# sanazkaviani/3d-latent-diffusion-model

Hardware: AMD Instinct MI355X
Metric: UNet denoising steps/sec (bf16, 1x4x24x24x24 latent; whole job = sum over GPUs) (higher is better)
Workload: dtype bf16

## Files before the change

3d-latent-diffusion-model_amd/csrc/ldm3d.hip:

```cpp
#include <hip/hip_runtime.h>
#include <dlfcn.h>
#include <math.h>
#include <stdarg.h>
#include <stdio.h>
#include <stdlib.h>
#include <string.h>

#include <algorithm>
#include <atomic>
#include <map>
#include <memory>
#include <string>
#include <vector>

#include "../../include/ldm3d.h"
#include "attention.h"
#include "conv_igemm.h"
#include "conv_halo.h"
#ifdef LDM_EXPERIMENTS
#include "conv_halo_pp.h"
#include "conv_halo_rw.h"
#endif
#include "conv_thin.h"
#include "gemm_light.h"
#include "gemm_light_x3.h"
#include "conv_block.h"
#include "conv_wgrad.h"
#include "conv_wgrad_w16.h"
#include "conv_wgrad_kw3.h"
#include "norm_elem.h"
#include "fin_gn.h"
#include "f32_path.h"
#include "f32_train.h"

#ifndef CONV_STAGES
#define CONV_STAGES 4
#endif

static thread_local char g_err[1024] = "";
static int fail(int code, const char* fmt, ...) {
    va_list ap; va_start(ap, fmt); vsnprintf(g_err, sizeof g_err, fmt, ap); va_end(ap);
    return code;
}
#define HIP_TRY(x) do { hipError_t e_ = (x); if (e_ != hipSuccess) \
    return fail(LDM_ERR_HIP, "%s failed: %s (%s:%d)", #x, hipGetErrorString(e_), __FILE__, __LINE__); } while (0)
#define LDM_TRY(x) do { int r_ = (x); if (r_ != 0) return r_; } while (0)


#ifdef LDM_EXPERIMENTS
static int g_block_slots = 0;
#endif
// ... 66 lines not shown
struct Ref { int base = BASE_NULL; size_t off = 0; };
static inline Ref ws_ref(size_t off) { Ref r; r.base = BASE_WS; r.off = off; return r; }
static inline Ref w_ref(size_t off) { Ref r; r.base = BASE_W; r.off = off; return r; }
static inline Ref io_ref(int i) { Ref r; r.base = BASE_IO0 + i; r.off = 0; return r; }
static inline Ref w32_ref(size_t off) { Ref r; r.base = BASE_W32; r.off = 2 * off; return r; }

struct Act {
    size_t off = 0; int C = 0; int N = 0, D = 0, H = 0, W = 0; bool valid = false;
    size_t stats_off = 0; bool has_stats = false;
    int stats_nrb = 0;
    int esz = 2;
    bool hl = false;
    size_t cs_off = 0; int cs_rows = 0;
    size_t bytes() const { return (size_t)N * D * H * W * C * esz; }
    long rows() const { return (long)N * D * H * W; }
};

enum OpKind { OP_PACK, OP_CONV, OP_FINALIZE, OP_GN_STATS, OP_GN_FINALIZE, OP_GN_PREP, OP_GN_APPLY, OP_ATTN, OP_SINUSOID,
              OP_GEMV, OP_VAE_HEADS, OP_GN_FUSED,
              OP_WT, OP_WT_BATCH, OP_WGRAD, OP_EXPORT, OP_EXPORT_BATCH, OP_COLSUM, OP_GNB, OP_ATTN_BWD, OP_ADD, OP_SUMPOOL, OP_LIN_DX, OP_LIN_DW, OP_VAE_HEADS_BWD,
              OP_GEMM_LIGHT,
              OP_COLSUM_BATCH,
              OP_IM2COL,
              OP_PACK32, OP_CONV32, OP_FIN32, OP_GN_STATS32, OP_GN_APPLY32, OP_ATTN32, OP_GEMV32,
              OP_TAP,
              OP_BUCKET, OP_BUCKET_JOIN,
              OP_UPS_SPLIT32,
              OP_CONV_THIN,
              OP_FIN_GN,
              OP_GEMM_LIGHT32,
              OP_CONV_BLOCK,
              OP_TEMB_ROW };

struct ConvCfg { int wgm, wgn, bk, splitk; int halo = 0, mtps = 0, qps = 0; int slab_lg = 0; };

struct Op {
    OpKind kind;
    Ref r[14];
    int i[24];
    float f[2];
    ConvCfg cc;
};

struct Pool {
    struct Blk { size_t off, size; };
    std::vector<Blk> free_list;
    std::map<size_t, size_t> live;
    size_t top = 0, high = 0;
    size_t alloc(size_t bytes) {
        bytes = rup_sz(bytes, 256);
        for (size_t k = 0; k < free_list.size(); ++k)
            if (free_list[k].size >= bytes) {
                size_t off = free_list[k].off;
                if (free_list[k].size == bytes) free_list.erase(free_list.begin() + k);
                else { free_list[k].off += bytes; free_list[k].size -= bytes; }
                live[off] = bytes;
                return off;
            }
        size_t off = top; top += bytes; high = std::max(high, top); live[off] = bytes;
        return off;
    }
    void release(size_t off) {
        auto it = live.find(off); if (it == live.end()) return;
        Blk b{off, it->second}; live.erase(it);
        free_list.push_back(b);
        std::sort(free_list.begin(), free_list.end(), [](const Blk& a, const Blk& c) { return a.off < c.off; });
        for (size_t k = 0; k + 1 < free_list.size();)
// ... 209 lines not shown
        a.valid = false; a.has_stats = false;
    }
    bool train = false, recording = false;

    struct ConvArgs {
        Act xa, xb;
        const ConvW* w = nullptr;
        int k = 3, stride = 1, pad = 1, ups = 0;
        int Do = 0, Ho = 0, Wo = 0;
        Act g1a, g1b; const ConvW* w1 = nullptr;
        Ref temb; int temb_stride = 0;
        Act residual;
        bool f32_out = false; Ref out_ref; int cout_real = 0;
        bool want_stats = true;
        Ref w_over; bool no_bias = false; int exact = 0;
        int temb_row = -1;
        int f32_tag = 0;
    };
    struct Tape {
        int kind = 0;
        ConvArgs c; Act out; bool leaf_input = false;
        const GnW* g = nullptr; Act xa, xb; size_t ab_off = 0, mr_off = 0; int groups = 0; bool silu = false;
        Act qkv, o; size_t lse_off = 0; int head_ch = 64;
    };
    std::vector<Tape> tape;

    static bool halo_enabled() { return ldm_knob("LDM_CONV_HALO", 1) != 0; }
    static int tall_mode() { return ldm_xknob("LDM_HALO_TALL", 2); }
    static bool light_enabled() { return ldm_knob("LDM_GEMM_LIGHT", 1) != 0; }
    static bool two_wg_enabled() { return ldm_knob("LDM_IGEMM_2WG", 1) != 0; }
    static bool phase_enabled() { return ldm_knob("LDM_CONV_PHASE", 1) != 0; }
    static bool halo_skip_enabled() { static const int v = ldm_knob("LDM_HALO_SKIP", 1); return v != 0; }
    static bool halo_skip_split_enabled() { static const int v = ldm_knob("LDM_HALO_SKIP_SPLIT", 1); return v != 0; }
    static ConvCfg choose_cfg(long M, int cout_pad, int steps0, int bk, int halo_n = 0, long halo_dhw = 0, bool halo_only = false, int steps1 = 0) {
        ConvCfg best{2, 2, bk, 1}; double best_t = 1e30;
        const int steps = steps0 + steps1;
        const int rb = bk * 2;
        static const int splits[] = {1, 2, 3, 4, 6, 8, 9, 12, 16, 18, 24, 27, 32, 48, 64};
        for (int wgn = 1; wgn <= 4 && !halo_only; wgn *= 2) {
            const int bn = 64 * wgn, bm = 64 * (4 / wgn);
            if (cout_pad % bn) continue;
            const long tiles = ((M + bm - 1) / bm) * (cout_pad / bn);
            const double c_mfma = (double)bm * bn * bk * 2.0 / 4096.0;
            const double c_load = (double)(bm + bn) * rb / 28.0;
            const double c_step = std::max(c_mfma, c_load) + 60.0;
            for (int sk : splits) {
                if (sk > 1 && steps / sk < 6) break;
                const long nwg = tiles * sk;
                const int sps = (steps + sk - 1) / sk;
                const double rounds = ceil((double)nwg / 256.0);
                double t = rounds * (sps * c_step + 2500.0);
                if (sk > 1) t += 6000.0 + (double)M * cout_pad * 4.0 * sk * 2.0 / 2500.0;
                if (t < best_t) { best_t = t; best = ConvCfg{4 / wgn, wgn, bk, sk}; }
            }
        }
        if (halo_n > 0 && bk == 64 && cout_pad % 128 == 0 && halo_enabled()) {
            const int mtps = (int)((halo_dhw + 125) / 126), Q = steps0 / 3;
            const long tiles = (long)halo_n * mtps * (cout_pad / 128);
            const double c_mfma = 128.0 * 128.0 * 64.0 * 2.0 / 4096.0;
            const double c_load = (128.0 / 3.0 + 128.0) * 128.0 / 28.0;
            const double c_step = std::max(c_mfma, c_load) + 30.0;
            for (int sk : splits) {
                if (sk > 1 && Q / sk < 3) break;
                const int qps = (Q + sk - 1) / sk, skr = (Q + qps - 1) / qps;
                const long nwg = tiles * skr;
                const double rounds = ceil((double)nwg / 256.0);
// ... 283 lines not shown
                Op op{}; op.kind = OP_CONV_BLOCK;
                op.r[0] = ws_ref(a.xa.off); op.r[2] = a.w_over.base != BASE_NULL ? a.w_over : w_ref(w.w_off); op.r[6] = a.no_bias ? Ref() : w_ref(w.b_off); op.r[8] = a.temb;
                op.r[9] = a.residual.valid ? ws_ref(a.residual.off) : Ref(); op.r[10] = ws_ref(out.off); op.r[12] = out.has_stats ? ws_ref(out.stats_off) : Ref();
                op.i[0] = N; op.i[1] = a.Do; op.i[2] = a.Ho; op.i[3] = a.Wo; op.i[4] = cin0; op.i[5] = TH; op.i[6] = a.temb_stride;
                plan->ops.push_back(op);
                if (recording) { Tape t; t.kind = 0; t.c = a; t.out = out; tape.push_back(t); }
                return out;
            }
        }
        if (conv_block128_enabled() && a.k == 3 && a.stride == 1 && a.pad == 1 && a.ups == 0 && !a.exact && !a.xb.valid && !a.w1 && !a.f32_out &&
            w.cout_pad == 128 && rup(w.cout, 32) == 128 && cin0 <= conv_block128_max_cin() && a.xa.D == a.Do && a.xa.H == a.Ho && a.xa.W == a.Wo) {
            const int td = (a.Do + BLK_TD - 1) / BLK_TD, th = (a.Ho + 7) / 8, tw = (a.Wo + BLK_TW - 1) / BLK_TW;
            static const long min_blocks = ldm_knob("LDM_CONV_BLOCK128_MIN", 192L);
            static const long max_blocks = ldm_xknob("LDM_CONV_BLOCK128_MAX", 0L);
            const long tiles128 = (long)N * td * th * tw;
            if (tiles128 >= min_blocks && tiles128 <= (max_blocks > 0 ? max_blocks : (long)device_cus())) {
                Act out = new_act(N, a.Do, a.Ho, a.Wo, 128);
                if (a.want_stats) { out.stats_off = pool.alloc((size_t)N * td * th * tw * 128 * 2 * 4); out.has_stats = true; out.stats_nrb = td * th * tw; }
                Op op{}; op.kind = OP_CONV_BLOCK;
                op.r[0] = ws_ref(a.xa.off); op.r[2] = a.w_over.base != BASE_NULL ? a.w_over : w_ref(w.w_off); op.r[6] = a.no_bias ? Ref() : w_ref(w.b_off); op.r[8] = a.temb;
                op.r[9] = a.residual.valid ? ws_ref(a.residual.off) : Ref(); op.r[10] = ws_ref(out.off); op.r[12] = out.has_stats ? ws_ref(out.stats_off) : Ref();
                op.i[0] = N; op.i[1] = a.Do; op.i[2] = a.Ho; op.i[3] = a.Wo; op.i[4] = cin0; op.i[5] = 8; op.i[6] = a.temb_stride; op.i[7] = 128;
                plan->ops.push_back(op);
                if (recording) { Tape t; t.kind = 0; t.c = a; t.out = out; tape.push_back(t); }
                return out;
            }
        }
        const int taps = phase ? 8 : a.k * a.k * a.k;
        const bool halo_ok = a.k == 3 && a.stride == 1 && a.pad == 1 && a.ups == 0 && !a.exact && !a.xb.valid && (!a.w1 || (halo_skip_enabled() && bk == 64)) &&
                             a.xa.D == a.Do && a.xa.H == a.Ho && a.xa.W == a.Wo;
        int nchunk0 = cin0 / bk, nchunk1 = cin1 / bk;
        int steps0 = taps * nchunk0, steps1 = nchunk1;
        ConvCfg cc = choose_cfg(M, w.cout_pad, steps0, bk, halo_ok ? N : 0, (long)a.Do * a.Ho * a.Wo, false, steps1);
        const int bm = 64 * cc.wgm, bn = 64 * cc.wgn;
        const int couts = a.f32_out ? 0 : rup(w.cout, 32);
        const int mtiles_pp = (int)(((long)a.xa.D * a.xa.H * a.xa.W + bm - 1) / bm);
        if (!cc.halo && cc.bk == 64 && cc.wgm <= 2 && cc.splitk == 1 && two_wg_enabled() && steps0 + steps1 <= 64 &&
            (phase ? (long)N * 8 * mtiles_pp : (M + bm - 1) / bm) * (w.cout_pad / bn) >= 512) {
            cc.bk = 32; nchunk0 = cin0 / 32; nchunk1 = cin1 / 32; steps0 = taps * nchunk0; steps1 = nchunk1;
        }
        Act out;
        if (!a.f32_out) {
            out = new_act(N, a.Do, a.Ho, a.Wo, couts);
            if (a.want_stats) {
                const long dhwo = (long)a.Do * a.Ho * a.Wo;
                if (cc.splitk > 1) {
                    out.stats_off = pool.alloc((size_t)((M + 31) / 32) * couts * 2 * 4); out.has_stats = true; out.stats_nrb = 0;
                } else if (cc.halo) {
                    out.stats_off = pool.alloc((size_t)N * cc.mtps * couts * 2 * 4); out.has_stats = true; out.stats_nrb = cc.mtps;
                } else if (phase) {
                    out.stats_off = pool.alloc((size_t)N * 8 * mtiles_pp * couts * 2 * 4); out.has_stats = true; out.stats_nrb = 8 * mtiles_pp;
                } else if (N == 1 || dhwo % bm == 0) {
                    out.stats_off = pool.alloc((size_t)((M + bm - 1) / bm) * couts * 2 * 4); out.has_stats = true;
                    out.stats_nrb = (int)(N == 1 ? (M + bm - 1) / bm : dhwo / bm);
                }
            }
        }
        Op op{}; op.kind = OP_CONV; op.cc = cc;
        op.r[0] = ws_ref(a.xa.off); op.r[1] = a.xb.valid ? ws_ref(a.xb.off) : Ref();
        op.r[2] = a.w_over.base != BASE_NULL ? a.w_over : w_ref(phase ? w.wp_off : w.w_off);
        op.r[3] = a.w1 ? ws_ref(a.g1a.off) : Ref(); op.r[4] = (a.w1 && a.g1b.valid) ? ws_ref(a.g1b.off) : Ref();
        op.r[5] = a.w1 ? w_ref(a.w1->w_off) : Ref();
        op.r[6] = a.no_bias ? Ref() : w_ref(w.b_off); op.r[7] = a.w1 ? w_ref(a.w1->b_off) : Ref();
        op.r[8] = a.temb; op.r[9] = a.residual.valid ? ws_ref(a.residual.off) : Ref();
        op.r[10] = a.f32_out ? a.out_ref : ws_ref(out.off);
        op.r[11] = Ref();
// ... 1155 lines not shown
            HIP_TRY(hipFuncSetAttribute(reinterpret_cast<const void*>(&conv3_halo_rw_kernel<0>), hipFuncAttributeMaxDynamicSharedMemorySize, HRW_LDS));
            HIP_TRY(hipFuncSetAttribute(reinterpret_cast<const void*>(&conv3_halo_rw_kernel<64>), hipFuncAttributeMaxDynamicSharedMemorySize, HRW_LDS));
            HIP_TRY(hipFuncSetAttribute(reinterpret_cast<const void*>(&conv3_halo_rw_kernel<4>), hipFuncAttributeMaxDynamicSharedMemorySize, HRW_LDS));
            rw_attr = true;
        }
        if ((p.dbg & 124) == 64) { hipLaunchKernelGGL((conv3_halo_rw_kernel<64>), dim3(tiles), dim3(512), HRW_LDS, s, p); return 0; }
        if ((p.dbg & 124) == 4) { hipLaunchKernelGGL((conv3_halo_rw_kernel<4>), dim3(tiles), dim3(512), HRW_LDS, s, p); return 0; }
        hipLaunchKernelGGL((conv3_halo_rw_kernel<0>), dim3(tiles), dim3(512), HRW_LDS, s, p);
        return 0;
    }
#endif
    if (p.dbg & (4 | 8 | 16 | 32 | 64 | 128 | 256)) {
#define ABL_CASE(A) if ((p.dbg & 508) == A) { \
            HIP_TRY(hipFuncSetAttribute(reinterpret_cast<const void*>(&conv3_halo_kernel<6, A>), hipFuncAttributeMaxDynamicSharedMemorySize, LDS)); \
            hipLaunchKernelGGL((conv3_halo_kernel<6, A>), dim3(p.mtiles * p.ntiles * p.splitk), dim3(512), LDS, s, p); return 0; }
        if ((p.dbg & 508) == 384) {
            constexpr int LDSX = LDS + 64;
            if (p.dbg & 2048) {
                HIP_TRY(hipFuncSetAttribute(reinterpret_cast<const void*>(&conv3_halo_kernel<6, 385>), hipFuncAttributeMaxDynamicSharedMemorySize, LDSX));
                hipLaunchKernelGGL((conv3_halo_kernel<6, 385>), dim3(p.mtiles * p.ntiles * p.splitk), dim3(512), LDSX, s, p); return 0;
            }
            HIP_TRY(hipFuncSetAttribute(reinterpret_cast<const void*>(&conv3_halo_kernel<6, 384>), hipFuncAttributeMaxDynamicSharedMemorySize, LDSX));
            hipLaunchKernelGGL((conv3_halo_kernel<6, 384>), dim3(p.mtiles * p.ntiles * p.splitk), dim3(512), LDSX, s, p); return 0;
        }
        ABL_CASE(4) ABL_CASE(8) ABL_CASE(16) ABL_CASE(12) ABL_CASE(20) ABL_CASE(24) ABL_CASE(32) ABL_CASE(40) ABL_CASE(84) ABL_CASE(68) ABL_CASE(64) ABL_CASE(128) ABL_CASE(256)
#undef ABL_CASE
    }
    if (loop) hipLaunchKernelGGL((conv3_halo_kernel<6, 0, false, true>), dim3(grid), dim3(512), LDS, s, p);
    else if (mi) hipLaunchKernelGGL((conv3_halo_kernel<6, 0, false, false, true>), dim3(grid), dim3(512), LDS, s, p);
    else hipLaunchKernelGGL((conv3_halo_kernel<6>), dim3(grid), dim3(512), LDS, s, p);
    return 0;
}

static int launch_conv_impl(const ConvParams& p, const ConvCfg& cc, hipStream_t s) {
    if (cc.halo) return launch_conv_halo(p, s, cc.halo == 2);
#define CASE(M_, N_, K_) if (cc.wgm == M_ && cc.wgn == N_ && cc.bk == K_) return launch_conv_t<M_, N_, K_>(p, s);
    CASE(2, 2, 64) CASE(4, 1, 64) CASE(1, 4, 64) CASE(2, 2, 32) CASE(4, 1, 32) CASE(1, 4, 32)
#undef CASE
    return fail(LDM_ERR_BAD_ARG, "no conv kernel for tile config %dx%d bk %d", cc.wgm, cc.wgn, cc.bk);
}

static inline int grid_for(long total, int per_block = 256, int cap = 4096) {
    long g = (total + per_block - 1) / per_block; if (g > cap) g = cap; if (g < 1) g = 1; return (int)g;
}

static void conv32_cfg(long M, int cout_pad, int steps, bool x3, int* bn_out, int* sk_out) {
    static const int f32_bn = ldm_knob("LDM_F32_BN", 0);
    static const int f32_wgs = ldm_knob("LDM_F32_WGS", 512);
    const int mtiles = (int)((M + 127) / 128);
    int bn = (cout_pad % 128) ? 64 : 128;
    if (f32_bn == 64 || (f32_bn == 1 && (long)mtiles * (cout_pad / 128) < 256)) bn = 64;
    const long tiles = (long)mtiles * ((cout_pad + bn - 1) / bn);
    int sk = 1;
    if (tiles < f32_wgs * 3 / 4) {
        sk = (int)std::min<long>(std::max<long>(1, f32_wgs / tiles), std::max(1, steps / (x3 ? 4 : 8)));
        const int sps = (steps + sk - 1) / sk; sk = (steps + sps - 1) / sps;
    }
    *bn_out = bn; *sk_out = sk;
}
static int fin32_stats_blocks(int N, int dhwo, int couts, int* rows) {
    const int cvec = couts / 4, rows_par = std::max(1, 256 / cvec);
    int nrb = std::min((dhwo + rows_par - 1) / rows_par, std::max(1, 256 / N));
    *rows = (dhwo + nrb - 1) / nrb;
    return (dhwo + *rows - 1) / *rows;
}
static void launch_conv32(const Conv32Params& p, bool x3, int bn, hipStream_t s) {
    const dim3 grid(p.mtiles * p.ntiles * p.splitk);
// ... 89 lines not shown
    static const int w16 = ldm_knob("LDM_WGRAD_W16", 1);
    if (w16 && p.pair == 0) {
        static bool attr16_tab[32] = {}; bool& attr16 = attr_flag(attr16_tab);
        if (!attr16) { HIP_TRY(hipFuncSetAttribute(reinterpret_cast<const void*>(&conv_wgrad_w16_kernel<0>), hipFuncAttributeMaxDynamicSharedMemorySize, LDS)); attr16 = true; }
        hipLaunchKernelGGL(conv_wgrad_w16_kernel<0>, dim3(p.co_tiles * p.ci_tiles * tg_ * p.ksplit), dim3(1024), LDS, s, p);
        return 0;
    }
    hipLaunchKernelGGL(conv_wgrad_kernel<0>, dim3(p.co_tiles * p.ci_tiles * tg_ * p.ksplit), dim3(512), LDS, s, p);
    return 0;
}

static bool wt_stores() { static const int v = ldm_xknob("LDM_WT_STORES", 1); return v != 0; }

struct PlanTrace { bool on = false; std::string path; PlanTrace() { const char* e = getenv("LDM_PLAN_TRACE"); if (e && *e) { on = true; path = e; } } };
static PlanTrace g_plan_trace;
struct LaneCtx { GradSyncState* sync = nullptr; };

static int run_plan(const Plan& plan, const Bases& bs, const int* rt, hipStream_t s, size_t begin = 0, size_t end = (size_t)-1,
                    LaneCtx lanes = LaneCtx()) {
    if (end > plan.ops.size()) end = plan.ops.size();
    const char* trace_path = g_plan_trace.on ? g_plan_trace.path.c_str() : nullptr;
    std::vector<hipEvent_t> tev;
    if (trace_path) { tev.resize(end - begin + 1); for (auto& e : tev) HIP_TRY(hipEventCreate(&e)); }
    struct TraceDone {
        const Plan& plan; size_t begin, end; std::vector<hipEvent_t>& ev; hipStream_t s; const char* path;
        ~TraceDone() {
            if (ev.empty()) return;
            (void)hipEventRecord(ev.back(), s); (void)hipEventSynchronize(ev.back());
            FILE* f = fopen(path, "a");
            for (size_t oi = begin; oi < end && f; ++oi) {
                const Op& o = plan.ops[oi]; float ms = 0.f; (void)hipEventElapsedTime(&ms, ev[oi - begin], ev[oi - begin + 1]);
                fprintf(f, "%zu,%zu,%d,%.3f", plan.ops.size(), oi, (int)o.kind, ms * 1e3f);
                if (o.kind == OP_CONV || o.kind == OP_FINALIZE)
                    fprintf(f, ",M=%d k=%d s=%d ups=%d cin=%d+%d(x%d) cin1=%d couts=%d cfg=%dx%dx%d splitk=%d halo=%d mtps=%d qps=%d", o.i[15], o.i[11], o.i[12],
                            o.i[14], o.i[0], o.i[1], o.i[19], o.i[2] + o.i[3], o.i[16], o.cc.wgm, o.cc.wgn, o.cc.bk, o.cc.splitk, o.cc.halo, o.cc.mtps, o.cc.qps);
                else fprintf(f, ",i=%d %d %d %d %d %d", o.i[0], o.i[1], o.i[2], o.i[3], o.i[4], o.i[5]);
                fprintf(f, "\n");
            }
            if (f) fclose(f);
            for (auto e : ev) (void)hipEventDestroy(e);
        }
    } trace_done{plan, begin, end, tev, s, trace_path};
    for (size_t oi = begin; oi < end; ++oi) {
        const Op& o = plan.ops[oi];
        const int* i = o.i;
        if (trace_path) HIP_TRY(hipEventRecord(tev[oi - begin], s));
        switch (o.kind) {
            case OP_PACK: {
                const long total = (long)i[0] * i[3] * i[2];
                int cx = rt[0], cc = rt[1];
                if (i[4]) { cx = i[1]; cc = 0; }
                if (cx + cc != i[1]) return fail(LDM_ERR_BAD_ARG, "x_channels + cond_channels = %d, model expects %d", cx + cc, i[1]);
                hipLaunchKernelGGL(pack2_ncdhw_kernel, dim3(grid_for(total)), dim3(256), 0, s, (const float*)rp(bs, o.r[0]), cx,
                                   (const float*)rp(bs, o.r[1]), cc, (bf16_t*)rp(bs, o.r[2]), i[0], i[2], i[3]);
                break; }
            case OP_IM2COL: {
                int cx = rt[0], cc = rt[1];
                if (i[6]) { cx = i[1]; cc = 0; }
                if (cx + cc != i[1]) return fail(LDM_ERR_BAD_ARG, "x_channels + cond_channels = %d, model expects %d", cx + cc, i[1]);
                const long total = (long)i[0] * i[3] * i[4] * i[5] * (i[2] / 8);
                hipLaunchKernelGGL(pack_im2col_kernel, dim3(grid_for(total, 256, 16384)), dim3(256), 0, s, (const float*)rp(bs, o.r[0]), cx,
                                   (const float*)rp(bs, o.r[1]), cc, (bf16_t*)rp(bs, o.r[2]), i[0], i[3], i[4], i[5], i[2]);
                break; }
            case OP_CONV_THIN: {
                ThinParams q{}; q.x = (const bf16_t*)rp(bs, o.r[0]); q.w = (const bf16_t*)rp(bs, o.r[2]); q.bias = (const float*)rp(bs, o.r[6]);
                q.out = (float*)rp(bs, o.r[10]); q.N = i[0]; q.D = i[1]; q.H = i[2]; q.W = i[3]; q.Cin = i[4]; q.CoutPad = i[5]; q.CoutReal = i[6];
                q.x3_c = i[7];
                if (!q.w) return fail(LDM_ERR_NOT_LOADED, "the weight arena is empty");
// ... 1129 lines not shown
    for (auto& e : g_prof.ev) HIP_TRY(hipEventCreate(&e));
    g_prof.wgm = wgm; g_prof.wgn = wgn; g_prof.bk = bk & 0xff; g_prof.halo = (bk >> 8) & 1; g_prof.on = true;
    return 0;
}
int ldm_profile_detail(double* flops, double* ms, int max) {
    if (!flops || !ms || max < 0) return fail(LDM_ERR_BAD_ARG, "null argument");
    const int n = (int)(g_prof.used / 2);
    for (int k = 0; k < n && k < max; ++k) {
        HIP_TRY(hipEventSynchronize(g_prof.ev[2 * k + 1]));
        float t = 0.f; HIP_TRY(hipEventElapsedTime(&t, g_prof.ev[2 * k], g_prof.ev[2 * k + 1]));
        flops[k] = g_prof.flops[k]; ms[k] = t;
    }
    return n;
}
int ldm_profile_stop(double out[5]) {
    if (!out) return fail(LDM_ERR_BAD_ARG, "null out");
    g_prof.on = false;
    double ms = 0.0, fl = 0.0;
    for (size_t k = 0; k + 1 < g_prof.used + 1 && k < g_prof.used; k += 2) {
        HIP_TRY(hipEventSynchronize(g_prof.ev[k + 1]));
        float t = 0.f; HIP_TRY(hipEventElapsedTime(&t, g_prof.ev[k], g_prof.ev[k + 1]));
        ms += t; fl += g_prof.flops[k / 2];
    }
    out[0] = (double)(g_prof.used / 2); out[1] = ms; out[2] = fl; out[3] = (double)g_prof.launches_all; out[4] = g_prof.flops_all;
    for (auto e : g_prof.ev) (void)hipEventDestroy(e);
    g_prof.ev.clear(); g_prof.used = 0; g_prof.flops.clear();
    return 0;
}
int ldm_model_plan_conv_cfgs(ldm_model* m, const char* kind, int B, int D, int H, int W, int* cfgs, int max_convs) {
    if (!m || !kind) return fail(LDM_ERR_BAD_ARG, "null argument");
    std::shared_ptr<Plan> p; LDM_TRY(get_plan(m, kind, B, D, H, W, &p));
    int n = 0;
    for (const Op& o : p->ops) if (o.kind == OP_CONV) {
        if (cfgs && n < max_convs) { cfgs[4 * n] = o.cc.wgm; cfgs[4 * n + 1] = o.cc.wgn; cfgs[4 * n + 2] = o.cc.bk | (o.cc.halo << 8); cfgs[4 * n + 3] = o.cc.splitk; }
        ++n;
    } else if (o.kind == OP_CONV_BLOCK) {
        if (cfgs && n < max_convs) { cfgs[4 * n] = 4; cfgs[4 * n + 1] = o.i[7] == 128 ? 2 : 1; cfgs[4 * n + 2] = 32 | ((o.i[7] == 128 ? 4 : 3) << 8); cfgs[4 * n + 3] = 1; }
        ++n;
    }
    return n;
}

int ldm_model_plan_launches(ldm_model* m, const char* kind, int B, int D, int H, int W) {
    if (!m || !kind) return fail(LDM_ERR_BAD_ARG, "null argument");
    std::shared_ptr<Plan> p; LDM_TRY(get_plan(m, kind, B, D, H, W, &p));
    int n = 0;
    for (const Op& o : p->ops) if (o.kind != OP_TAP) ++n;
    return n;
}

static char* g_zero_page = nullptr;
static int ensure_zero_page() {
    if (g_zero_page) return 0;
    HIP_TRY(hipMalloc((void**)&g_zero_page, 8192));
    HIP_TRY(hipMemset(g_zero_page, 0, 8192));
    HIP_TRY(hipDeviceSynchronize());
    return 0;
}

int ldm_op_conv3d_block128(const void* x, int cin, const void* w, const float* bias, const float* temb, int temb_stride, const void* residual,
                           void* out, float* stats, int N, int D, int H, int W, void* stream) {
    if (!x || !w || !out || N < 1 || D < 1 || H < 1 || W < 1 || cin < 32 || cin % 32) return fail(LDM_ERR_BAD_ARG, "bad argument");
    if ((long)N * D * H * W * cin * 2 >= (1L << 32)) return fail(LDM_ERR_BAD_ARG, "the input tensor exceeds 4 GiB (split the batch)");
    BlockParams q{}; q.x = (const bf16_t*)x; q.w = (const bf16_t*)w; q.bias = bias; q.temb = temb; q.temb_stride = temb_stride;
    q.residual = (const bf16_t*)residual; q.out = (bf16_t*)out; q.stats = stats; q.N = N; q.D = D; q.H = H; q.W = W; q.Cin = cin;
    HIP_TRY(launch_conv_block128(q, (hipStream_t)stream));
    return 0;
// ... 41 lines not shown
    int bk = 64;
    if (ca % 64 || cb % 64 || c1a % 64 || c1b % 64) bk = 32;
    const int Du = Din << ups, Hu = Hin << ups, Wu = Win << ups;
    const int pad_total = (stride == 2 && pad == 0 && ksize == 3) ? 1 : 2 * pad;
    const int Do = (Du + pad_total - ksize) / stride + 1, Ho = (Hu + pad_total - ksize) / stride + 1,
              Wo = (Wu + pad_total - ksize) / stride + 1;
    const long M = (long)N * Do * Ho * Wo;
    if (M >= (1L << 31) || M < 1) return fail(LDM_ERR_BAD_ARG, "bad output size");
    if (!stats && !wgn && !splitk && out_bf16 && !out_f32 && gemm_light_ok(ksize, stride, ups, cin0, cin1 == 0, !temb && !bias2) &&
        Builder::light_enabled() && M * (long)cin0 * 2 < (1L << 31)) {
        LightParams lp{}; lp.x = (const bf16_t*)xa; lp.w = (const bf16_t*)w; lp.bias = bias; lp.residual = (const bf16_t*)residual;
        lp.out = (bf16_t*)out_bf16; lp.stats = nullptr; lp.M = (int)M; lp.K = cin0; lp.CoutS = rup(cout, 32);
        lp.xb = (const bf16_t*)xb; lp.ca = ca;
        HIP_TRY(launch_gemm_light(lp, cout_pad, gemm_light_big(M, cout_pad), (hipStream_t)stream));
        return 0;
    }
    const int taps = ksize * ksize * ksize;
    ConvParams p{};
    p.x0a = (const bf16_t*)xa; p.x0b = (const bf16_t*)xb; p.c0a = ca; p.c0b = cb; p.w0 = (const bf16_t*)w;
    p.x1a = (const bf16_t*)x1a; p.x1b = (const bf16_t*)x1b; p.c1a = c1a; p.c1b = c1b; p.w1 = (const bf16_t*)w1;
    p.zero_page = (const bf16_t*)g_zero_page;
    p.N = N; p.Din = Din; p.Hin = Hin; p.Win = Win; p.Dout = Do; p.Hout = Ho; p.Wout = Wo;
    p.ksize = ksize; p.stride = stride; p.pad = pad; p.ups = ups; p.exact = exact; p.M = (int)M;
    p.CoutS = rup(cout, 32); p.CoutPad = cout_pad; p.CoutReal = cout;
    p.nchunk0 = cin0 / bk; p.nchunk1 = cin1 / bk; p.steps0 = taps * p.nchunk0; p.steps1 = p.nchunk1;
    const bool halo_ok = ksize == 3 && stride == 1 && pad == 1 && ups == 0 && !exact && cb == 0 && bk == 64 &&
                         (cin1 == 0 || (Builder::halo_skip_enabled() && (splitk <= 1 || Builder::halo_skip_split_enabled()))) && Builder::halo_enabled();
    ConvCfg cc = Builder::choose_cfg(M, cout_pad, p.steps0, bk, halo_ok ? N : 0, (long)Do * Ho * Wo, false, p.steps1);
    if (wgn) {
        if ((wgn != 1 && wgn != 2 && wgn != 4) || cout_pad % (64 * wgn)) return fail(LDM_ERR_BAD_ARG, "bad wgn");
        cc.wgn = wgn; cc.wgm = 4 / wgn; cc.halo = (wgn == 2 && halo_ok && cout_pad % 128 == 0) ? 1 : (wgn == 1 && halo_ok && Builder::tall_mode() != 0) ? 2 : 0;
    }
    if (splitk) cc.splitk = splitk;
    if (cc.splitk < 1 || cc.splitk > p.steps0 + p.steps1) return fail(LDM_ERR_BAD_ARG, "bad splitk");
    if (cc.halo) {
        const int Q = 9 * p.nchunk0;
        if (cc.splitk > Q) cc.splitk = Q;
        cc.qps = (Q + cc.splitk - 1) / cc.splitk; cc.splitk = (Q + cc.qps - 1) / cc.qps;
        cc.mtps = (int)(((long)Do * Ho * Wo + (cc.halo == 2 ? 253 : 125)) / (cc.halo == 2 ? 254 : 126));
    }
    p.splitk = cc.splitk; p.steps_per_split = cc.halo ? 3 * cc.qps : (p.steps0 + p.steps1 + cc.splitk - 1) / cc.splitk;
    p.halo_mtps = cc.mtps; p.q_per_split = cc.qps;
    p.mtiles = cc.halo ? N * cc.mtps : (int)((M + 64 * cc.wgm - 1) / (64 * cc.wgm)); p.ntiles = cout_pad / (64 * cc.wgn);
    p.bias = bias; p.bias2 = bias2; p.temb = temb; p.temb_stride = temb_stride; p.residual = (const bf16_t*)residual;
    p.out = out_f32 ? nullptr : (bf16_t*)out_bf16; p.out_f32 = out_f32;
    if (cc.splitk > 1) {
        const size_t need = (size_t)cc.splitk * M * cout_pad * 4;
        if (!scratch || scratch_bytes < need) return fail(LDM_ERR_WORKSPACE, "split-K scratch too small: need %zu bytes", need);
        p.partial = (float*)scratch;
    }
    if (stats) {
        const long dhwo = (long)Do * Ho * Wo; const int bm = 64 * cc.wgm;
        if (out_f32 || !stats_nrb) return fail(LDM_ERR_BAD_ARG, "statistics need the bf16 output form");
        if (cc.splitk > 1) { if (N > 1 && dhwo % 32) return fail(LDM_ERR_UNSUPPORTED, "statistics: DHW %% 32 != 0 with a batch"); *stats_nrb = (int)(N == 1 ? (M + 31) / 32 : dhwo / 32); }
        else if (cc.halo) *stats_nrb = cc.mtps;
        else { if (N > 1 && dhwo % bm) return fail(LDM_ERR_UNSUPPORTED, "statistics: tiles straddle samples"); *stats_nrb = (int)(N == 1 ? (M + bm - 1) / bm : dhwo / bm); }
        p.stats = stats;
    }
    p.dbg = (int)ldm_xknob("LDM_CONV_DBG", 0);
    if (p.dbg & 512) {
        if (cc.splitk > 1 || !scratch || scratch_bytes < (size_t)p.mtiles * p.ntiles * (64 + 4096)) return fail(LDM_ERR_BAD_ARG, "stamps need scratch and splitk 1");
        p.stamps = (unsigned long long*)scratch;
    }
    if (fg && cc.splitk > 1) p.slab_lg = fg->lg;
    LDM_TRY(launch_conv(p, cc, (hipStream_t)stream));
    if (cc.splitk > 1) {
        FinalizeParams f{}; f.partial = p.partial; f.splitk = p.splitk; f.M = p.M; f.CoutPad = p.CoutPad; f.CoutS = p.CoutS;
        f.CoutReal = p.CoutReal; f.DHWo = Do * Ho * Wo; f.bias = bias; f.bias2 = bias2; f.temb = temb; f.temb_stride = temb_stride;
// ... 768 lines not shown
```

Baseline: 492.9.

## Add whole-cube split-K conv kernel for tiny 3D volumes (edge at most 6)

Adds a specialized 3x3x3 conv kernel for tiny spatial volumes (at most 6^3). Each workgroup loads the whole zero-padded cube for one 64-channel input slice plus all 27 taps of weights into LDS in a single pass. It then runs all taps from LDS, adds any skip-input GEMM, and writes split-K partials. It targets the bottleneck-resolution convs, where the generic igemm/halo tiling leaves most of each tile empty and pays repeated load stalls. In exchange it needs a split-K finalize pass over an fp32 partial buffer, and runs one workgroup per CU with a large LDS footprint.

```diff
diff --git a/3d-latent-diffusion-model_amd/csrc/conv_cube.h b/3d-latent-diffusion-model_amd/csrc/conv_cube.h
--- /dev/null
+++ b/3d-latent-diffusion-model_amd/csrc/conv_cube.h
@@ -0,0 +1,171 @@
+#pragma once
+#include "conv_igemm.h"
+
+constexpr int CUBE_EDGE = 6;
+constexpr int CUBE_RP = 7, CUBE_PP = 49;
+constexpr int CUBE_ROWS = 448;
+constexpr int CUBE_TILES = 16;
+constexpr int CUBE_WOFF = 8 * CUBE_ROWS * 16;
+constexpr int CUBE_SOFF = CUBE_WOFF + 27 * 2048;
+constexpr int CUBE_SWOFF = CUBE_SOFF + 8 * 256 * 16;
+constexpr int CUBE_LDS = CUBE_SWOFF + 2048;
+static_assert(CUBE_LDS <= 160 * 1024, "LDS budget");
+static_assert(CUBE_ROWS % 64 == 0 && CUBE_ROWS % 16 == 0, "whole LDS-DMA copies; chunk stride a multiple of 16 rows");
+
+__device__ __forceinline__ void cube_vm_wait(int n) {
+    switch (n) {
+    case 0: asm volatile("s_waitcnt vmcnt(0)" ::: "memory"); break;
+    case 8: asm volatile("s_waitcnt vmcnt(8)" ::: "memory"); break;
+    case 9: asm volatile("s_waitcnt vmcnt(9)" ::: "memory"); break;
+    default: asm volatile("s_waitcnt vmcnt(0)" ::: "memory"); break;
+    }
+}
+__device__ __forceinline__ void cube_barrier() {
+    asm volatile("s_waitcnt lgkmcnt(0)" ::: "memory");
+    __builtin_amdgcn_s_barrier();
+    asm volatile("" ::: "memory");
+}
+
+__global__ __launch_bounds__(256, 1) __attribute__((amdgpu_waves_per_eu(1, 1))) void conv3_cube_kernel(const ConvParams p) {
+#if defined(__HIP_DEVICE_COMPILE__)
+    extern __shared__ __attribute__((aligned(16))) char smem[];
+    typedef __attribute__((address_space(3))) void* lds_ptr_t;
+    constexpr unsigned OOB = 0x80000000u;
+    KSTAMP_BEGIN(12);
+    const int tid = threadIdx.x, lane = tid & 63;
+    const int wave = __builtin_amdgcn_readfirstlane(tid >> 6);
+    const int split = blockIdx.x, n0 = blockIdx.y * 16, smp = blockIdx.z;
+    const int D = p.Dout, H = p.Hout, W = p.Wout, DHW = D * H * W, dom = D * H * CUBE_RP;
+    const unsigned cin2 = (unsigned)p.c0a * 2u, ci2 = (unsigned)split * 128u;
+
+    {
+        __amdgpu_buffer_rsrc_t rs_w = __builtin_amdgcn_make_buffer_rsrc((void*)p.w0, 0, (int)(27u * (unsigned)p.CoutPad * cin2), 0x00020000);
+        const int co = lane & 15, cq = lane >> 4;
+        for (int u = wave; u < 54; u += 4) {
+            const int tap = u >> 1, ch = (u & 1) * 4 + cq;
+            const unsigned vo = (unsigned)(tap * p.CoutPad + n0 + co) * cin2 + ci2 + (unsigned)ch * 16u;
+            __builtin_amdgcn_raw_ptr_buffer_load_lds(rs_w, (lds_ptr_t)(smem + CUBE_WOFF + u * 1024), 16, vo, 0, 0, 0);
+        }
+    }
+    {
+        const bf16_t* xs = p.x0a + (size_t)smp * DHW * p.c0a;
+        __amdgpu_buffer_rsrc_t rs_x = __builtin_amdgcn_make_buffer_rsrc((void*)xs, 0, (int)((unsigned)DHW * cin2), 0x00020000);
+        for (int v = wave; v < 8 * (CUBE_ROWS / 64); v += 4) {
+            const int ch = v / (CUBE_ROWS / 64), r = (v - ch * (CUBE_ROWS / 64)) * 64 + lane;
+            const int dp = r / CUBE_PP, rem = r - dp * CUBE_PP, hp = rem / CUBE_RP, wp = rem - hp * CUBE_RP;
+            const bool real = dp >= 1 && dp <= D && hp >= 1 && hp <= H && wp >= 1 && wp <= W;
+            const unsigned vo = real ? (unsigned)(((dp - 1) * H + hp - 1) * W + wp - 1) * cin2 + ci2 + (unsigned)ch * 16u : OOB;
+            __builtin_amdgcn_raw_ptr_buffer_load_lds(rs_x, (lds_ptr_t)(smem + ch * (CUBE_ROWS * 16) + (v - ch * (CUBE_ROWS / 64)) * 1024), 16, vo, 0, 0, 0);
+        }
+    }
+    int j0 = 0, j1 = 0;
+    if (p.steps1 > 0) {
+        const int per = (p.steps1 + p.splitk - 1) / p.splitk;
+        j0 = split * per; j1 = j0 + per; if (j1 > p.steps1) j1 = p.steps1; if (j0 > j1) j0 = j1;
+    }
+    unsigned s_vox = OOB;
+    {
+        const int q = wave * 64 + lane;
+        if (q < dom) {
+            const int d = q / (H * CUBE_RP), rem = q - d * H * CUBE_RP, h = rem / CUBE_RP, w = rem - h * CUBE_RP;
+            if (w < W) s_vox = (unsigned)((d * H + h) * W + w);
+        }
+    }
+    const int nca = p.c1a / 64;
+    const unsigned w1row2 = (unsigned)(p.c1a + p.c1b) * 2u;
+    auto issue_skip = [&](const int j) {
+        const bool a = j < nca;
+        const bf16_t* src = (a ? p.x1a : p.x1b) + (size_t)smp * DHW * (a ? p.c1a : p.c1b);
+        const unsigned row2 = (unsigned)(a ? p.c1a : p.c1b) * 2u, jc = (unsigned)(a ? j : j - nca) * 128u;
+        __amdgpu_buffer_rsrc_t rs_s = __builtin_amdgcn_make_buffer_rsrc((void*)src, 0, (int)((unsigned)DHW * row2), 0x00020000);
+#pragma unroll
+        for (int i = 0; i < 8; ++i) {
+            const unsigned vo = s_vox != OOB ? s_vox * row2 + jc + (unsigned)i * 16u : OOB;
+            __builtin_amdgcn_raw_ptr_buffer_load_lds(rs_s, (lds_ptr_t)(smem + CUBE_SOFF + i * 4096 + wave * 1024), 16, vo, 0, 0, 0);
+        }
+        if (wave < 2) {
+            __amdgpu_buffer_rsrc_t rs_1w = __builtin_amdgcn_make_buffer_rsrc((void*)p.w1, 0, (int)((unsigned)p.CoutPad * w1row2), 0x00020000);
+            const unsigned vo = (unsigned)(n0 + (lane & 15)) * w1row2 + (unsigned)j * 128u + (unsigned)(wave * 4 + (lane >> 4)) * 16u;
+            __builtin_amdgcn_raw_ptr_buffer_load_lds(rs_1w, (lds_ptr_t)(smem + CUBE_SWOFF + wave * 1024), 16, vo, 0, 0, 0);
+        }
+    };
+    const bool has_skip = j1 > j0;
+    if (has_skip) issue_skip(j0);
+    const int skip_copies = 8 + (wave < 2 ? 1 : 0);
+
+    const int mh = wave & 1, kh = wave >> 1;
+    const int fr = lane & 15, ch = kh * 4 + (lane >> 4);
+    int abase[8];
+#pragma unroll
+    for (int t = 0; t < 8; ++t) {
+        const int q = (mh * 8 + t) * 16 + fr;
+        int row = 0;
+        if (q < dom) {
+            const int d = q / (H * CUBE_RP), rem = q - d * H * CUBE_RP, h = rem / CUBE_RP, w = rem - h * CUBE_RP;
+            row = d * CUBE_PP + h * CUBE_RP + w;
+        }
+        abase[t] = ch * (CUBE_ROWS * 16) + row * 16;
+    }
+    const int wbase = CUBE_WOFF + ch * 256 + fr * 16;
+    f32x4 acc[8];
+#pragma unroll
+    for (int t = 0; t < 8; ++t) acc[t] = (f32x4){0.f, 0.f, 0.f, 0.f};
+
+    cube_vm_wait(has_skip ? skip_copies : 0);
+    cube_barrier();
+    KSTAMP(1);
+    bf16x8 wf[2], af[2][8];
+    wf[0] = *reinterpret_cast<const bf16x8*>(smem + wbase);
+#pragma unroll
+    for (int t = 0; t < 8; ++t) af[0][t] = *reinterpret_cast<const bf16x8*>(smem + abase[t]);
+#pragma unroll
+    for (int tap = 0; tap < 27; ++tap) {
+        const int cur = tap & 1, nxt = cur ^ 1;
+        if (tap + 1 < 27) {
+            const int k = tap + 1, off = ((k / 9) * CUBE_PP + ((k / 3) % 3) * CUBE_RP + k % 3) * 16;
+            wf[nxt] = *reinterpret_cast<const bf16x8*>(smem + wbase + k * 2048);
+#pragma unroll
+            for (int t = 0; t < 8; ++t) af[nxt][t] = *reinterpret_cast<const bf16x8*>(smem + abase[t] + off);
+        }
+#pragma unroll
+        for (int t = 0; t < 8; ++t) acc[t] = __builtin_amdgcn_mfma_f32_16x16x32_bf16(wf[cur], af[cur][t], acc[t], 0, 0, 0);
+#pragma unroll
+        for (int t = 0; t < 8; ++t) { __builtin_amdgcn_sched_group_barrier(0x008, 1, 0); __builtin_amdgcn_sched_group_barrier(0x100, 1, 0); }
+        __builtin_amdgcn_sched_group_barrier(0x100, 1, 0);
+    }
+    for (int j = j0; j < j1; ++j) {
+        if (j > j0) { cube_barrier(); issue_skip(j); }
+        asm volatile("s_waitcnt vmcnt(0)" ::: "memory");
+        cube_barrier();
+        const bf16x8 sw = *reinterpret_cast<const bf16x8*>(smem + CUBE_SWOFF + ch * 256 + fr * 16);
+#pragma unroll
+        for (int t = 0; t < 8; ++t) {
+            const bf16x8 sa = *reinterpret_cast<const bf16x8*>(smem + CUBE_SOFF + ch * 4096 + ((mh * 8 + t) * 16 + fr) * 16);
+            acc[t] = __builtin_amdgcn_mfma_f32_16x16x32_bf16(sw, sa, acc[t], 0, 0, 0);
+        }
+    }
+    KSTAMP(2);
+    cube_barrier();
+    float4* xch = reinterpret_cast<float4*>(smem);
+    if (kh == 1) {
+#pragma unroll
+        for (int t = 0; t < 8; ++t) xch[(mh * 8 + t) * 64 + lane] = make_float4(acc[t][0], acc[t][1], acc[t][2], acc[t][3]);
+    }
+    cube_barrier();
+    if (kh == 0) {
+        const int c = n0 + 4 * (lane >> 4);
+#pragma unroll
+        for (int t = 0; t < 8; ++t) {
+            const int q = (mh * 8 + t) * 16 + fr;
+            if (q >= dom) continue;
+            const int d = q / (H * CUBE_RP), rem = q - d * H * CUBE_RP, h = rem / CUBE_RP, w = rem - h * CUBE_RP;
+            if (w >= W) continue;
+            const float4 o = xch[(mh * 8 + t) * 64 + lane];
+            const int m = smp * DHW + (d * H + h) * W + w;
+            *reinterpret_cast<float4*>(slab_ptr(p.partial, split, p.M, p.CoutPad, p.slab_lg, m, c)) =
+                make_float4(acc[t][0] + o.x, acc[t][1] + o.y, acc[t][2] + o.z, acc[t][3] + o.w);
+        }
+    }
+    KSTAMP_DRAIN(3);
+#endif
+}
diff --git a/3d-latent-diffusion-model_amd/csrc/ldm3d.hip b/3d-latent-diffusion-model_amd/csrc/ldm3d.hip
--- a/3d-latent-diffusion-model_amd/csrc/ldm3d.hip
+++ b/3d-latent-diffusion-model_amd/csrc/ldm3d.hip
@@ -17,6 +17,7 @@
 #include "attention.h"
 #include "conv_igemm.h"
 #include "conv_halo.h"
+#include "conv_cube.h"
 #ifdef LDM_EXPERIMENTS
 #include "conv_halo_pp.h"
 #include "conv_halo_rw.h"
@@ -149,7 +150,7 @@
               OP_CONV_BLOCK,
               OP_TEMB_ROW };
 
-struct ConvCfg { int wgm, wgn, bk, splitk; int halo = 0, mtps = 0, qps = 0; int slab_lg = 0; };
+struct ConvCfg { int wgm, wgn, bk, splitk; int halo = 0, mtps = 0, qps = 0; int slab_lg = 0; int cube = 0; };
 
 struct Op {
     OpKind kind;
@@ -425,6 +426,12 @@
     static bool phase_enabled() { return ldm_knob("LDM_CONV_PHASE", 1) != 0; }
     static bool halo_skip_enabled() { static const int v = ldm_knob("LDM_HALO_SKIP", 1); return v != 0; }
     static bool halo_skip_split_enabled() { static const int v = ldm_knob("LDM_HALO_SKIP_SPLIT", 1); return v != 0; }
+    static bool cube_enabled() { return ldm_knob("LDM_CONV_CUBE", 1) != 0; }
+    static bool cube_ok(int D, int H, int W, int cin0, int c1a, int c1b, int cout_pad) {
+        return cube_enabled() && D >= 1 && H >= 1 && W >= 1 && D <= CUBE_EDGE && H <= CUBE_EDGE && W <= CUBE_EDGE && cin0 % 64 == 0 && cin0 >= 128 &&
+               c1a % 64 == 0 && c1b % 64 == 0 && cout_pad % 16 == 0;
+    }
+    static ConvCfg cube_cfg(int cin0) { ConvCfg c{2, 2, 64, cin0 / 64}; c.cube = 1; return c; }
     static ConvCfg choose_cfg(long M, int cout_pad, int steps0, int bk, int halo_n = 0, long halo_dhw = 0, bool halo_only = false, int steps1 = 0) {
         ConvCfg best{2, 2, bk, 1}; double best_t = 1e30;
         const int steps = steps0 + steps1;
@@ -774,6 +781,8 @@
         int nchunk0 = cin0 / bk, nchunk1 = cin1 / bk;
         int steps0 = taps * nchunk0, steps1 = nchunk1;
         ConvCfg cc = choose_cfg(M, w.cout_pad, steps0, bk, halo_ok ? N : 0, (long)a.Do * a.Ho * a.Wo, false, steps1);
+        if (halo_ok && bk == 64 && !hp && !train && !phase && cube_ok(a.Do, a.Ho, a.Wo, cin0, a.w1 ? a.g1a.C : 0, (a.w1 && a.g1b.valid) ? a.g1b.C : 0, w.cout_pad))
+            cc = cube_cfg(cin0);
         const int bm = 64 * cc.wgm, bn = 64 * cc.wgn;
         const int couts = a.f32_out ? 0 : rup(w.cout, 32);
         const int mtiles_pp = (int)(((long)a.xa.D * a.xa.H * a.xa.W + bm - 1) / bm);
@@ -1995,7 +2004,20 @@
     return 0;
 }
 
+static int launch_conv_cube(const ConvParams& p, hipStream_t s) {
+    if (p.c0a % 64 || p.x0b || p.x3_n || p.splitk != p.c0a / 64 || p.splitk < 2 || p.CoutPad % 16 || p.Dout > CUBE_EDGE || p.Hout > CUBE_EDGE ||
+        p.Wout > CUBE_EDGE || p.c1a % 64 || p.c1b % 64 || !p.partial)
+        return fail(LDM_ERR_BAD_ARG, "conv3_cube_kernel: unsupported conv (cin %d, splitk %d, %dx%dx%d)", p.c0a, p.splitk, p.Dout, p.Hout, p.Wout);
+    static bool attr_tab[32] = {}; bool& attr_set = attr_flag(attr_tab);
+    if (!attr_set) {
+        HIP_TRY(hipFuncSetAttribute(reinterpret_cast<const void*>(&conv3_cube_kernel), hipFuncAttributeMaxDynamicSharedMemorySize, CUBE_LDS));
+        attr_set = true;
+    }
+    hipLaunchKernelGGL(conv3_cube_kernel, dim3(p.splitk, p.CoutPad / 16, p.N), dim3(256), CUBE_LDS, s, p);
+    return 0;
+}
 static int launch_conv_impl(const ConvParams& p, const ConvCfg& cc, hipStream_t s) {
+    if (cc.cube) return launch_conv_cube(p, s);
     if (cc.halo) return launch_conv_halo(p, s, cc.halo == 2);
 #define CASE(M_, N_, K_) if (cc.wgm == M_ && cc.wgn == N_ && cc.bk == K_) return launch_conv_t<M_, N_, K_>(p, s);
     CASE(2, 2, 64) CASE(4, 1, 64) CASE(1, 4, 64) CASE(2, 2, 32) CASE(4, 1, 32) CASE(1, 4, 32)
@@ -2151,8 +2173,8 @@
                 const Op& o = plan.ops[oi]; float ms = 0.f; (void)hipEventElapsedTime(&ms, ev[oi - begin], ev[oi - begin + 1]);
                 fprintf(f, "%zu,%zu,%d,%.3f", plan.ops.size(), oi, (int)o.kind, ms * 1e3f);
                 if (o.kind == OP_CONV || o.kind == OP_FINALIZE)
-                    fprintf(f, ",M=%d k=%d s=%d ups=%d cin=%d+%d(x%d) cin1=%d couts=%d cfg=%dx%dx%d splitk=%d halo=%d mtps=%d qps=%d", o.i[15], o.i[11], o.i[12],
-                            o.i[14], o.i[0], o.i[1], o.i[19], o.i[2] + o.i[3], o.i[16], o.cc.wgm, o.cc.wgn, o.cc.bk, o.cc.splitk, o.cc.halo, o.cc.mtps, o.cc.qps);
+                    fprintf(f, ",M=%d k=%d s=%d ups=%d cin=%d+%d(x%d) cin1=%d couts=%d cfg=%dx%dx%d splitk=%d halo=%d mtps=%d qps=%d cube=%d", o.i[15], o.i[11], o.i[12],
+                            o.i[14], o.i[0], o.i[1], o.i[19], o.i[2] + o.i[3], o.i[16], o.cc.wgm, o.cc.wgn, o.cc.bk, o.cc.splitk, o.cc.halo, o.cc.mtps, o.cc.qps, o.cc.cube);
                 else fprintf(f, ",i=%d %d %d %d %d %d", o.i[0], o.i[1], o.i[2], o.i[3], o.i[4], o.i[5]);
                 fprintf(f, "\n");
             }
@@ -3348,7 +3370,7 @@
     std::shared_ptr<Plan> p; LDM_TRY(get_plan(m, kind, B, D, H, W, &p));
     int n = 0;
     for (const Op& o : p->ops) if (o.kind == OP_CONV) {
-        if (cfgs && n < max_convs) { cfgs[4 * n] = o.cc.wgm; cfgs[4 * n + 1] = o.cc.wgn; cfgs[4 * n + 2] = o.cc.bk | (o.cc.halo << 8); cfgs[4 * n + 3] = o.cc.splitk; }
+        if (cfgs && n < max_convs) { cfgs[4 * n] = o.cc.wgm; cfgs[4 * n + 1] = o.cc.wgn; cfgs[4 * n + 2] = o.cc.bk | ((o.cc.cube ? 5 : o.cc.halo) << 8); cfgs[4 * n + 3] = o.cc.splitk; }
         ++n;
     } else if (o.kind == OP_CONV_BLOCK) {
         if (cfgs && n < max_convs) { cfgs[4 * n] = 4; cfgs[4 * n + 1] = o.i[7] == 128 ? 2 : 1; cfgs[4 * n + 2] = 32 | ((o.i[7] == 128 ? 4 : 3) << 8); cfgs[4 * n + 3] = 1; }
@@ -3456,8 +3478,10 @@
         cc.wgn = wgn; cc.wgm = 4 / wgn; cc.halo = (wgn == 2 && halo_ok && cout_pad % 128 == 0) ? 1 : (wgn == 1 && halo_ok && Builder::tall_mode() != 0) ? 2 : 0;
     }
     if (splitk) cc.splitk = splitk;
+    if (!wgn && !splitk && halo_ok && !out_f32 && !(ldm_xknob("LDM_CONV_DBG", 0)) && Builder::cube_ok(Do, Ho, Wo, cin0, c1a, c1b, cout_pad))
+        cc = Builder::cube_cfg(cin0);
     if (cc.splitk < 1 || cc.splitk > p.steps0 + p.steps1) return fail(LDM_ERR_BAD_ARG, "bad splitk");
-    if (cc.halo) {
+    if (cc.halo && !cc.cube) {
         const int Q = 9 * p.nchunk0;
         if (cc.splitk > Q) cc.splitk = Q;
         cc.qps = (Q + cc.splitk - 1) / cc.splitk; cc.splitk = (Q + cc.qps - 1) / cc.qps;
```

Result: faster. 509.0 (median of 6 runs) (+3.3%).
